# usamec/GAML

Hardware: NVIDIA B200
Metric: alignments_scored_per_s (higher is better)
Workload: dtype f64

## Files before the change

### gaml_b200/csrc/engine.cu

```cuda
#include <cuda_runtime.h>
#include <dlfcn.h>

#include <algorithm>
#include <atomic>
#include <climits>
#include <limits>
#include <cmath>
#include <cstdio>
#include <chrono>
#include <cstring>
#include <memory>
#include <memory_resource>
#include <string>
#include <unordered_map>
#include <unordered_set>
#include <vector>

#include "../../include/gaml_b200.h"
#include "kernels.h"
#include "walk_set.h"

namespace gaml {
namespace {

// ... 950 lines not shown
        CU(rs.d_pairs.reserve((size_t)rs.n_local * 16, 0, false, ctx->stream));
        uint32_t* bad = static_cast<uint32_t*>(ctx->d_csr_temp.p);
        CU(cudaMemsetAsync(bad, 0, 4, ctx->stream));
        launch_pack_pairs(rs.mate[0].first.p, rs.mate[1].first.p, rs.n_local, rs.d_partner12.as<int32_t>(), rs.d_pairs.p, bad, ctx->stream);
        launches++;
        pack_bad = 1;
        CU(cudaMemcpyAsync(&pack_bad, bad, 4, cudaMemcpyDeviceToHost, ctx->stream));
      }
      CU(cudaStreamSynchronize(ctx->stream));
      if (rs.cfg.kind == GAML_KIND_PAIRED && rs.n_mates == 2 && rs.n_local > 0) rs.pairs_ok = pack_bad == 0;
      rs.fast_ok = false;
      if (rs.pairs_ok && rs.comb_ok && rs.lens_uniform && rs.tq_shift > 0) {
        CU(rs.d_fast.reserve((size_t)rs.n_local * 16, 0, false, ctx->stream));
        CU(rs.d_xlist.reserve((size_t)rs.n_local * 4, 0, false, ctx->stream));
        uint32_t* flags = rs.mate[0].cursor.as<uint32_t>();
        CU(build_fast_pairs(rs.d_pairs.p, rs.n_local, rs.tq_shift, rs.ins_n, rs.uniform_ll, rs.d_fast.p, flags, rs.d_xlist.as<uint32_t>(),
                            ctx->d_csr_temp.p, ctx->d_csr_temp.cap, ctx->stream, &launches));
        uint32_t n_cross = 0;
        CU(cudaMemcpyAsync(&n_cross, flags + rs.n_local, 4, cudaMemcpyDeviceToHost, ctx->stream));
        CU(cudaStreamSynchronize(ctx->stream));
        rs.n_cross = (int)n_cross;
        rs.fast_ok = true;
      }
      rs.t2pack_ok = false;
      if (rs.pairs_ok && rs.class_begin[3] > 0) {
        const size_t n0 = (size_t)(rs.class_begin[1] - rs.class_begin[0]), n1 = (size_t)(rs.class_begin[2] - rs.class_begin[1]),
                     n2 = (size_t)(rs.class_begin[3] - rs.class_begin[2]);
        rs.t2base[0] = 0;
        rs.t2base[1] = (uint32_t)(2 * n0);
        rs.t2base[2] = (uint32_t)(2 * n0 + 2 * n1);
        CU(rs.d_t2pack.reserve((2 * n0 + 2 * n1 + 3 * n2) * 16, 0, false, ctx->stream));
        uint32_t* bad = static_cast<uint32_t*>(ctx->d_csr_temp.p);
        CU(cudaMemsetAsync(bad, 0, 4, ctx->stream));
        launch_pack_tier2(rs.d_cdesc.p, rs.mate[0].crows.p, rs.mate[1].crows.p, rs.class_begin, rs.cbase, rs.t2base, rs.d_t2pack.p,
                          bad, ctx->stream);
        launches++;
        uint32_t t2_bad = 1;
        CU(cudaMemcpyAsync(&t2_bad, bad, 4, cudaMemcpyDeviceToHost, ctx->stream));
        CU(cudaStreamSynchronize(ctx->stream));
        rs.t2pack_ok = t2_bad == 0;
      }
      ctx->stats.kernel_launches += launches;
      rs.complex_dirty = false;
      rs.base_built = false;
      if (rs.cfg.kind == GAML_KIND_PAIRED && rs.n_mates == 2 && rs.n_local > 0 && rs.pairs_ok) {
        DevBuf counts;
        CU(counts.reserve((size_t)rs.n_local * 2, 0, false, ctx->stream));
        for (int m = 0; m < 2; m++) {
          MateStore& st = rs.mate[m];
          launch_extract_counts(st.first.p, st.rowptr.as<uint32_t>(), rs.n_local, counts.as<uint16_t>(), ctx->stream);
          st.h_count.resize((size_t)rs.n_local);
          CU(cudaMemcpyAsync(st.h_count.data(), counts.p, (size_t)rs.n_local * 2, cudaMemcpyDeviceToHost, ctx->stream));
          CU(cudaStreamSynchronize(ctx->stream));
          ctx->stats.kernel_launches++;
        }
        CU(rs.d_dirty.reserve((size_t)rs.n_local * 4, 0, false, ctx->stream));
        CU(cudaMemsetAsync(rs.d_dirty.p, 0, (size_t)rs.n_local * 4, ctx->stream));
        rs.h_dirty.assign((size_t)rs.n_local, 0);
        rs.n_appx = 0;
        rs.base_built = true;
      }
    }
    if (pass == 1 || !rs.fast_ok || rs.perm_valid || !ctx->permute_reads) break;
    {
      const int n = rs.n_local;
      DevBuf keys, ids, inv, temp, nf;
      CU(keys.reserve((size_t)n * 2 * 8, 0, false, ctx->stream));
      CU(ids.reserve((size_t)n * 2 * 4, 0, false, ctx->stream));
// ... 2793 lines not shown
```

### gaml_b200/csrc/kernels.cu

```cuda
#include <cub/device/device_radix_sort.cuh>
#include <cub/device/device_scan.cuh>

#include <chrono>
#include <cstdio>
#include <cstdlib>
#include <cstring>
#include <type_traits>
#include <utility>

#include "kernels.h"

namespace gaml {

namespace {

constexpr int kCapLong = 8;
constexpr int kBlock = 256;
constexpr int kOvfBlock = 128;

__device__ __forceinline__ int4 ldg4(const void* p) { return __ldg(reinterpret_cast<const int4*>(p)); }
__device__ __forceinline__ uint4 ldg_stream(const uint4* p) {
  uint4 v;
  asm volatile("ld.global.nc.L1::no_allocate.v4.u32 {%0,%1,%2,%3}, [%4];" : "=r"(v.x), "=r"(v.y), "=r"(v.z), "=r"(v.w) : "l"(p));
  return v;
}
__device__ __forceinline__ void ldg256(const uint4* p, uint4& a, uint4& b) {
  asm volatile("ld.global.nc.v8.u32 {%0,%1,%2,%3,%4,%5,%6,%7}, [%8];"
               : "=r"(a.x), "=r"(a.y), "=r"(a.z), "=r"(a.w), "=r"(b.x), "=r"(b.y), "=r"(b.z), "=r"(b.w) : "l"(p));
}
constexpr int kPackKeyBits = 22;
constexpr uint32_t kPackKeyMask = (1u << kPackKeyBits) - 1u;
constexpr uint32_t kPackEdMask = 0x7fu;

__device__ __forceinline__ int wrap_add(int a, int b) { return (int)((unsigned)a + (unsigned)b); }

__device__ __forceinline__ void pdl_release() { asm volatile("griddepcontrol.launch_dependents;"); }
__device__ __forceinline__ void pdl_wait() { asm volatile("griddepcontrol.wait;" ::: "memory"); }
enum { kTlApply = 0, kTlTier1, kTlTier2, kTlOverflow, kTlDelta, kTlTotal, kTlKernels };
__device__ __forceinline__ unsigned long long global_ns() {
  unsigned long long t;
  asm volatile("mov.u64 %0, %%globaltimer;" : "=l"(t));
  return t;
}
__device__ __forceinline__ void tl_begin(unsigned long long* tl, int k) {
  if (tl && threadIdx.x == 0) atomicMax(tl + 2 * k, ~global_ns());
}
__device__ __forceinline__ void tl_end(unsigned long long* tl, int k) {
  if (tl && threadIdx.x == 0) atomicMax(tl + 2 * k + 1, global_ns());
}
__device__ __forceinline__ void prefetch_l2(const void* p) { asm volatile("prefetch.global.L2 [%0];" ::"l"(p)); }

constexpr double kFixScale = 1099511627776.0;
constexpr double kFixLimit = 4194304.0;

struct Acc {
  unsigned long long lo;
  long long hi;
  unsigned neginf, bad;
};
__device__ __forceinline__ Acc acc_zero() { return Acc{0ull, 0ll, 0u, 0u}; }
__device__ __forceinline__ void acc_add_q(Acc& a, long long q) {
// ... 654 lines not shown
  const RowShort* rows1 = static_cast<const RowShort*>(P.m[0].crows);
  const RowShort* rows2 = static_cast<const RowShort*>(P.m[1].crows);
  const int n_tiles = (P.n_main + kBlock - 1) / kBlock;
  int tile = blockIdx.x, buf = 0;
  for (; tile < n_tiles; __syncthreads(), tile = s_tile[buf], buf ^= 1) {
    if (threadIdx.x == 0) s_tile[buf] = (int)gridDim.x + (int)atomicAdd(P.tile_counter + 2, 1u);
    const int k = tile * kBlock + (int)threadIdx.x;
    if (k >= P.n_main) continue;
    int cls = 0;
#pragma unroll
    for (int c = 1; c < 5; c++) cls += (k >= P.class_begin[c]) ? 1 : 0;
    const uint32_t j = (uint32_t)(k - P.class_begin[cls]);
    const int4 dsc = ldg4(static_cast<const int4*>(P.cdesc) + k);
    const int r = dsc.x;
    const uint32_t ll = (uint32_t)dsc.y;
    double acc;
    int st;
    switch (cls) {
      case 0: st = tier2_read<1, 2>(P, rows1, rows2, P.cbase[0][0] + j, P.cbase[1][0] + 2 * j, ll, acc); break;
      case 1: st = tier2_read<2, 1>(P, rows1, rows2, P.cbase[0][1] + 2 * j, P.cbase[1][1] + j, ll, acc); break;
      case 2: st = tier2_read<2, 2>(P, rows1, rows2, P.cbase[0][2] + 2 * j, P.cbase[1][2] + 2 * j, ll, acc); break;
      default: st = 1; acc = 0.0; break;
    }
    if (P.dirty && __ldg(P.dirty + r)) continue;
    if (st > 0) {
      P.values[r] = acc;
      acc_read(P, sum, floored, acc, (ll & 0xffff) + (ll >> 16));
    } else if (st < 0) {
      push_overflow(P, r);
    }
  }
}

struct Rec8 { uint32_t w; int pos; };
__device__ __forceinline__ Rec8 rec8(uint32_t a, uint32_t b) { return Rec8{a, (int)b}; }

template <int N1, int N2>
__device__ __forceinline__ int tier2_packed_read(const ScoreParams& P, const int4* __restrict__ sa1, const int4* __restrict__ sa2,
                                                 const Rec8 (&x)[2], const Rec8 (&y)[2], uint32_t ll, double& acc, long long& qv) {
  const int l1 = ll & 0xffff, l2 = ll >> 16;
  int4 ox[2], oy[2];
#pragma unroll
  for (int i = 0; i < 2; i++) {
    ox[i] = __ldg(sa1 + (x[i < N1 ? i : 0].w & kPackKeyMask));
    oy[i] = __ldg(sa2 + (y[i < N2 ? i : 0].w & kPackKeyMask));
  }
  int ex[2], ey[2];
#pragma unroll
  for (int i = 0; i < 2; i++) {
    ex[i] = (int)((x[i < N1 ? i : 0].w >> kPackKeyBits) & kPackEdMask);
    ey[i] = (int)((y[i < N2 ? i : 0].w >> kPackKeyBits) & kPackEdMask);
  }
  const TermEntry* __restrict__ tq = P.tq ? static_cast<const TermEntry*>(P.tq) + 1 : nullptr;
  double px[2], py[2];
  if (!tq) {
#pragma unroll
    for (int i = 0; i < 2; i++) {
      px[i] = __dmul_rn(__ldg(P.m[0].pow_mismatch + ex[i]), __ldg(P.m[0].pow_match + (l1 - ex[i])));
      py[i] = __dmul_rn(__ldg(P.m[1].pow_mismatch + ey[i]), __ldg(P.m[1].pow_match + (l2 - ey[i])));
    }
  }
  bool lx[2], ly[2], multi = false;
  int wx[2], wy[2], qx[2], qy[2], orx[2], ory[2];
#pragma unroll
  for (int i = 0; i < 2; i++) {
    const uint32_t fx = (uint32_t)ox[i].x, fy = (uint32_t)oy[i].x;
    const bool hx = i < N1, hy = i < N2;
    const bool vx = hx && (fx & 0x7fffffffu) == P.epoch, vy = hy && (fy & 0x7fffffffu) == P.epoch;
    multi |= (vx && (fx >> 31)) || (vy && (fy >> 31));
    wx[i] = ox[i].y; wy[i] = oy[i].y;
    qx[i] = wrap_add(x[hx ? i : 0].pos, ox[i].z); qy[i] = wrap_add(y[hy ? i : 0].pos, oy[i].z);
    lx[i] = vx && qx[i] >= ox[i].w;
    ly[i] = vy && qy[i] >= oy[i].w;
    orx[i] = (int)((x[hx ? i : 0].w >> 29) & 1u); ory[i] = (int)((y[hy ? i : 0].w >> 29) & 1u);
  }
  bool order = false;
  if (N1 > 1) {
    const bool dup = lx[0] && lx[1] && wx[0] == wx[1] && qx[0] == qx[1];
    const bool same = ((x[0].w ^ x[1].w) >> kPackKeyBits) == 0u;
    order |= dup && !same;
    lx[1] = lx[1] && !dup;
  }
  if (N2 > 1) {
    const bool dup = ly[0] && ly[1] && wy[0] == wy[1] && qy[0] == qy[1];
    const bool same = ((y[0].w ^ y[1].w) >> kPackKeyBits) == 0u;
    order |= dup && !same;
    ly[1] = ly[1] && !dup;
  }
  bool ok[2][2];
  int dist[2][2];
  int nt = 0, nok = 0;
#pragma unroll
  for (int i = 0; i < N1; i++) {
#pragma unroll
    for (int j = 0; j < N2; j++) {
      const bool fwd = qx[i] < qy[j];
      const int d = fwd ? qy[j] - qx[i] + l2 : qx[i] - qy[j] + l1;
      const bool term = lx[i] && ly[j] && wx[i] == wy[j] && orx[i] != ory[j] && orx[i] == (fwd ? 0 : 1);
      nt += term ? 1 : 0;
      ok[i][j] = term && (unsigned)d < (unsigned)P.ins_n;
      nok += ok[i][j] ? 1 : 0;
      dist[i][j] = ok[i][j] ? d : 0;
    }
  }
  double t[2][2];
  long long tqv[2][2];
  if (tq) {
    const int lim = 1 << P.tq_shift;
    bool untab = false;
    TermEntry e[2][2];
#pragma unroll
    for (int i = 0; i < N1; i++) {
#pragma unroll
      for (int j = 0; j < N2; j++) {
        const bool fit = ex[i] < lim && ey[j] < lim;
        untab |= ok[i][j] && !fit;
        const size_t idx = fit ? (size_t)((ex[i] << P.tq_shift) | ey[j]) * (size_t)P.ins_n + (size_t)dist[i][j] : 0;
        const int4 w = __ldg(reinterpret_cast<const int4*>(tq + idx));
        e[i][j].t = __hiloint2double(w.y, w.x);
        e[i][j].q = (long long)(((unsigned long long)(uint32_t)w.w << 32) | (uint32_t)w.z);
      }
    }
#pragma unroll
    for (int i = 0; i < N1; i++) {
#pragma unroll
      for (int j = 0; j < N2; j++) { t[i][j] = e[i][j].t; tqv[i][j] = e[i][j].q; }
    }
    if (untab) {
#pragma unroll
      for (int i = 0; i < N1; i++) {
#pragma unroll
        for (int j = 0; j < N2; j++) {
          if (ok[i][j] && !(ex[i] < lim && ey[j] < lim)) {
            t[i][j] = __dmul_rn(__dmul_rn(__ldg(P.uni_prob[0] + ex[i]), __ldg(P.uni_prob[1] + ey[j])), __ldg(P.ins_tab + dist[i][j]));
            tqv[i][j] = kTermOdd;
          }
        }
      }
    }
  } else {
#pragma unroll
    for (int i = 0; i < N1; i++) {
#pragma unroll
      for (int j = 0; j < N2; j++) {
        t[i][j] = __dmul_rn(__dmul_rn(px[i], py[j]), __ldg(P.ins_tab + dist[i][j]));
        tqv[i][j] = kTermOdd;
      }
    }
  }
  acc = 0.0;
  qv = kTermOdd;
#pragma unroll
  for (int i = 0; i < N1; i++) {
#pragma unroll
    for (int j = 0; j < N2; j++) {
      acc = __dadd_rn(acc, ok[i][j] ? t[i][j] : 0.0);
      if (ok[i][j] && nok == 1) qv = tqv[i][j];
    }
  }
  return multi ? 0 : ((order || nt > 2) ? -1 : 1);
}

__device__ __forceinline__ void acc_term_known(Acc& a, unsigned& floored, const double2* log_tab, double p, long long qv,
                                               double pstar, long long qthr) {
  if (p < pstar) {
    floored++;
    acc_add_q(a, qthr);
  } else if (qv != kTermOdd) {
    acc_add_q(a, qv);
  } else {
    const double lg = table_log(log_tab, p);
    if (fabs(lg) < kFixLimit) acc_add_q(a, __double2ll_rn(lg * kFixScale));
    else acc_count_odd(a, lg);
  }
}

__device__ __forceinline__ void tier2_packed_tiles(const ScoreParams& P, int* s_tile, Acc& sum, unsigned& floored) {
  const int4* sa1 = reinterpret_cast<const int4*>(P.m[0].slots_a);
  const int4* sa2 = reinterpret_cast<const int4*>(P.m[1].slots_a);
  const double2* log_tab = static_cast<const double2*>(P.log_tab);
  const uint4* __restrict__ pk = static_cast<const uint4*>(P.t2pack);
  const int n_tiles = (P.n_main + kBlock - 1) / kBlock;
  int tile = blockIdx.x, buf = 0;
  for (; tile < n_tiles; __syncthreads(), tile = s_tile[buf], buf ^= 1) {
    if (threadIdx.x == 0) s_tile[buf] = (int)gridDim.x + (int)atomicAdd(P.tile_counter + 2, 1u);
    const int k = tile * kBlock + (int)threadIdx.x;
    if (k >= P.n_main) continue;
    int cls = 0;
#pragma unroll
    for (int c = 1; c < 5; c++) cls += (k >= P.class_begin[c]) ? 1 : 0;
    const uint32_t j = (uint32_t)(k - P.class_begin[cls]);
    int r, st;
    uint32_t ll;
    double acc = 0.0;
    long long qv = kTermOdd;
    if (cls < 3) {
      const uint32_t n_c = (uint32_t)(P.class_begin[cls + 1] - P.class_begin[cls]);
      const uint4* base = pk + P.t2base[cls];
      const uint4 u0 = ldg_stream(base + j), u1 = ldg_stream(base + n_c + j);
      r = (int)u0.x;
      ll = u0.y;
      if (cls == 0) {
        const Rec8 x[2] = {rec8(u0.z, u0.w), rec8(u0.z, u0.w)}, y[2] = {rec8(u1.x, u1.y), rec8(u1.z, u1.w)};
        st = tier2_packed_read<1, 2>(P, sa1, sa2, x, y, ll, acc, qv);
      } else if (cls == 1) {
        const Rec8 x[2] = {rec8(u1.x, u1.y), rec8(u1.z, u1.w)}, y[2] = {rec8(u0.z, u0.w), rec8(u0.z, u0.w)};
        st = tier2_packed_read<2, 1>(P, sa1, sa2, x, y, ll, acc, qv);
      } else {
        const uint4 u2 = ldg_stream(base + 2 * n_c + j);
        const Rec8 x[2] = {rec8(u1.x, u1.y), rec8(u1.z, u1.w)}, y[2] = {rec8(u2.x, u2.y), rec8(u2.z, u2.w)};
        st = tier2_packed_read<2, 2>(P, sa1, sa2, x, y, ll, acc, qv);
      }
    } else {
      const int4 dsc = ldg4(static_cast<const int4*>(P.cdesc) + k);
      r = dsc.x;
      ll = (uint32_t)dsc.y;
      st = 1;
    }
    if (P.dirty && __ldg(P.dirty + r)) continue;
    if (st > 0) {
      P.values[r] = acc;
      double pstar;
      long long qthr;
      term_consts(P, (ll & 0xffff) + (ll >> 16), pstar, qthr);
      acc_term_known(sum, floored, log_tab, acc, qv, pstar, qthr);
    } else if (st < 0) {
      push_overflow(P, r);
    }
  }
}

struct TwoLive { Placed1 p0, p1; int n; bool multi, order; };
__device__ __forceinline__ void two_live_scan(const ScoreParams& P, int m, const RowShort* __restrict__ rows, uint32_t b,
                                              uint32_t n, TwoLive& t) {
  t.n = 0;
  t.multi = t.order = false;
  t.p0 = t.p1 = Placed1{false, false, 0, 0, 0};
  for (uint32_t i = 0; i < n; i += 2) {
    const int4 r0 = ldg4(rows + b + i), r1 = i + 1 < n ? ldg4(rows + b + i + 1) : r0;
    Placed1 q[2] = {place_row(P, m, r0), place_row(P, m, r1)};
    if (i + 1 >= n) q[1].live = q[1].multi = false;
#pragma unroll
    for (int j = 0; j < 2; j++) {
      if (!q[j].live) continue;
      t.multi |= q[j].multi;
      if (t.n > 0 && t.p0.walk == q[j].walk && t.p0.pos == q[j].pos) {
        if (t.p0.edor != q[j].edor) t.order = true;
      } else if (t.n > 1 && t.p1.walk == q[j].walk && t.p1.pos == q[j].pos) {
        if (t.p1.edor != q[j].edor) t.order = true;
      } else if (t.n == 0) {
        t.p0 = q[j];
        t.n = 1;
      } else if (t.n == 1) {
        t.p1 = q[j];
        t.n = 2;
      } else {
        t.order = true;
      }
    }
  }
}
// ... 398 lines not shown
      __syncthreads();
#pragma unroll
      for (int j = 0; j < kR; j++) u_cur[j] = u_nxt[j];
      tile = next;
      next = s_tile[buf];
      buf ^= 1;
    }
  } else {
    while (tile < n_tiles) {
      if (threadIdx.x == 0) s_tile[buf] = 2 * (int)gridDim.x + (int)atomicAdd(P.tile_counter, 1u);
      prefetch_tile(next);
      tier1_body<kCov, kPacked, false, kR>(P, src1, src2, lane, sa1, sa2, log_tab, tile * kTile + wib * (32 * kR), n, sum, floored);
      __syncthreads();
      tile = next;
      next = s_tile[buf];
      buf ^= 1;
    }
  }
  if (kPhase != 1 && kTab && P.n_cross > 0) {
    const uint4* __restrict__ pairs = static_cast<const uint4*>(P.pairs);
    constexpr int kXR = 2, kXTile = kXR * kBlock;
    const int x_tiles = (P.n_cross + kXTile - 1) / kXTile;
    __syncthreads();
    int xt = blockIdx.x, xbuf = 0;
    for (; xt < x_tiles; __syncthreads(), xt = s_tile[xbuf], xbuf ^= 1) {
      if (threadIdx.x == 0) s_tile[xbuf] = (int)gridDim.x + (int)atomicAdd(P.tile_counter + 3, 1u);
      tier1_body<false, true, kTab, kXR>(P, pairs, src2, lane, sa1, sa2, log_tab, xt * kXTile + wib * (32 * kXR), P.n_cross, sum, floored, P.xlist);
    }
  }
  if (kPhase != 2) tl_end(P.timeline, kTlTier1);
  if (kPhase != 1 && P.n_main > 0) {
    __syncthreads();
    if (kPhase == 0) tl_begin(P.timeline, kTlTier2);
    if (!kCov && P.t2pack) tier2_packed_tiles(P, s_tile, sum, floored);
    else tier2_tiles(P, s_tile, sum, floored);
  }
  if (kPhase != 1) tl_end(P.timeline, kTlTier2);
  if (!P.chain_first) pdl_wait();
  block_accumulate(sum, floored, P.accum);
  if (P.finish_here) finish_set_if_complete(P);
}


__device__ __forceinline__ bool paired_read_any(const ScoreParams& P, int r, uint32_t ll, double& acc) {
  if (paired_read_ordered(P, r, acc)) return true;
  const int n1 = gather_short(P.m[0], P.epoch, r, nullptr), n2 = gather_short(P.m[1], P.epoch, r, nullptr);
  const unsigned long long base = atomicAdd(P.scratch_cursor, (unsigned long long)(n1 + n2));
  if (base + n1 + n2 > P.scratch_cap) {
    atomicOr(P.error_flag, 2u);
    return false;
  }
  Plc* a = P.scratch + base;
  Plc* b = a + n1;
  gather_short(P.m[0], P.epoch, r, a);
  gather_short(P.m[1], P.epoch, r, b);
  acc = apply_pairs(P, a, n1, b, n2, ll & 0xffff, ll >> 16, acc, P.n_erased);
  return true;
}

__global__ void __launch_bounds__(kOvfBlock) paired_multi_kernel(const ScoreParams P) {
  tl_begin(P.timeline, kTlDelta);
  if (P.chain_first) pdl_wait();
  pdl_release();
  Acc sum = acc_zero();
  unsigned floored = 0;
  const uint32_t total = P.n_mtouch > 0 ? __ldg(P.mtouch_prefix + P.n_mtouch) : 0u;
  for (uint32_t q = blockIdx.x * blockDim.x + threadIdx.x; q < total; q += gridDim.x * blockDim.x) {
// ... 1416 lines not shown
  batch_finalize_kernel<<<(B.n_cand + 127) / 128, 128, 0, st>>>(B, out, error_flag, (long long)P.n_reads);
  if (timing) {
    cudaEventRecord(ev[4], st);
    cudaEventSynchronize(ev[4]);
    float t[4];
    for (int i = 0; i < 4; i++) cudaEventElapsedTime(&t[i], ev[i], ev[i + 1]);
    fprintf(stderr, "[gaml_b200 batch] n_len %d: base %.3f ms, prefix %.3f ms, touch %.3f ms (%u records), finalize %.3f ms\n", B.n_len, t[0], t[1],
            t[2], n_touch_records, t[3]);
    for (auto& e : ev) cudaEventDestroy(e);
  }
}
int batch_hist_bins(int n_len) { return ((n_len + kBatchMaxLen - 1) / kBatchMaxLen) * (kBatchMaxLen + 1); }
int batch_launches(int n_len, bool touch) { return 2 * ((n_len + kBatchMaxLen - 1) / kBatchMaxLen) + (touch ? 1 : 0) + 1; }

__global__ void build_term_table_kernel(const double* p1, const double* p2, const double* ins, int ins_n, int shift, const double2* log_tab,
                                        TermEntry* out) {
  const size_t total = ((size_t)1 << (2 * shift)) * (size_t)ins_n;
  for (size_t i = blockIdx.x * (size_t)blockDim.x + threadIdx.x; i < total; i += (size_t)gridDim.x * blockDim.x) {
    const int d = (int)(i % (size_t)ins_n);
    const int ee = (int)(i / (size_t)ins_n);
    const int e1 = ee >> shift, e2 = ee & ((1 << shift) - 1);
    const double t = __dmul_rn(__dmul_rn(p1[e1], p2[e2]), ins[d]);
    out[i + 1] = TermEntry{t, fix_log(log_tab, t)};
    if (i == 0) out[0] = TermEntry{0.0, kTermOdd};
  }
}
void launch_build_term_table(const double* p1, const double* p2, const double* ins, int ins_n, int shift, const void* log_tab, void* out,
                             int sm_count, cudaStream_t st) {
  const size_t total = ((size_t)1 << (2 * shift)) * (size_t)ins_n;
  build_term_table_kernel<<<grid_for(total, 256, sm_count, 8), 256, 0, st>>>(p1, p2, ins, ins_n, shift, static_cast<const double2*>(log_tab),
                                                                           static_cast<TermEntry*>(out));
}

__global__ void pack_fast_kernel(const uint4* pairs, int n, int shift, int ins_n, uint32_t uniform_ll, uint4* out, uint32_t* flags) {
  const int r = blockIdx.x * blockDim.x + threadIdx.x;
  if (r > n) return;
  if (r == n) { flags[r] = 0u; return; }
  const uint4 pr = pairs[r];
  const uint32_t key1 = pr.x & kPackKeyMask;
  const int e1 = (int)((pr.x >> kPackKeyBits) & kPackEdMask), e2 = (int)((pr.y >> kPackKeyBits) & kPackEdMask);
  const int xo = (int)((pr.x >> 29) & 1u), yo = (int)((pr.y >> 29) & 1u);
  const bool none = ((pr.x >> 30) & 1u) != 0u || ((pr.y >> 30) & 1u) != 0u;
  const bool tier2 = (pr.x >> 31) != 0u, same = (pr.y >> 31) != 0u;
  const int pos1 = (int)pr.z, pos2 = (int)pr.w;
  const int l1 = (int)(uniform_ll & 0xffff), l2 = (int)(uniform_ll >> 16);
  const bool fit = e1 < (1 << shift) && e2 < (1 << shift);
  uint4 v = make_uint4(0u, 0u, 0u, 0u);
  uint32_t cross = 0u;
  uint32_t tix = 0u;
  if (!none && same && fit) {
    const bool fwd = pos1 < pos2;
    const int d = fwd ? pos2 - pos1 + l2 : pos1 - pos2 + l1;
    const bool term = xo != yo && xo == (fwd ? 0 : 1) && (unsigned)d < (unsigned)ins_n;
    tix = term ? 1u + (uint32_t)((e1 << shift) | e2) * (uint32_t)ins_n + (uint32_t)d : 0u;
  }
  if (tier2) {
    v.x = 0x80000000u | key1;
    v.w = tix;
  } else if (none) {
    v.x = 0x40000000u;
  } else if (!same || !fit) {
    v.x = 0x80000000u | key1;
    cross = 1u;
  } else {
    v.x = key1;
    v.y = (uint32_t)pos1;
    v.z = (uint32_t)pos2;
    v.w = tix;
  }
  out[r] = v;
  flags[r] = cross;
}
__global__ void perm_keys_kernel(const uint4* fast, int n, unsigned long long* keys, uint32_t* ids) {
  const int r = blockIdx.x * blockDim.x + threadIdx.x;
  if (r >= n) return;
  const uint4 f = fast[r];
  const bool elsewhere = (f.x >> 31) != 0u, noterm = ((f.x >> 30) & 1u) != 0u;
  unsigned long long k;
  if (elsewhere) k = (1ull << 63) | ((unsigned long long)(f.x & 0x3fffffffu) << 32) | (unsigned long long)f.w;
  else if (noterm) k = (0x3fffffffull << 32) | (unsigned long long)(uint32_t)r;
  else k = ((unsigned long long)(f.x & 0x3fffffffu) << 32) | (unsigned long long)f.w;
  keys[r] = k;
  ids[r] = (uint32_t)r;
}
__global__ void perm_finish_kernel(const unsigned long long* sorted_keys, const uint32_t* sorted_ids, int n, uint32_t* inv, uint32_t* n_fast) {
  const int i = blockIdx.x * blockDim.x + threadIdx.x;
  if (i >= n) return;
  inv[sorted_ids[i]] = (uint32_t)i;
// ... 34 lines not shown
}
cudaError_t build_fast_pairs(const void* pairs, int n, int shift, int ins_n, uint32_t uniform_ll, void* fast, uint32_t* flags, uint32_t* list,
                             void* temp, size_t temp_bytes, cudaStream_t st, int* launches) {
  pack_fast_kernel<<<(n + 1 + 255) / 256, 256, 0, st>>>(static_cast<const uint4*>(pairs), n, shift, ins_n, uniform_ll, static_cast<uint4*>(fast), flags);
  size_t need = 0;
  cub::DeviceScan::ExclusiveSum(nullptr, need, flags, flags, n + 1, st);
  if (need > temp_bytes) return cudaErrorMemoryAllocation;
  cudaError_t err = cub::DeviceScan::ExclusiveSum(temp, need, flags, flags, n + 1, st);
  if (err != cudaSuccess) return err;
  scatter_flagged_kernel<<<(n + 255) / 256, 256, 0, st>>>(flags, n, list);
  (*launches) += 3;
  return cudaGetLastError();
}

__global__ void pack_pairs_kernel(const int4* first1, const int4* first2, int n, const int32_t* partner12, uint4* out, uint32_t* bad) {
  const int r = blockIdx.x * blockDim.x + threadIdx.x;
  if (r >= n) return;
  const int4 a = ldg4(first1 + r), b = ldg4(first2 + r);
  const bool none1 = a.x < 0, none2 = b.x < 0;
  const uint32_t k1 = none1 ? 0u : (uint32_t)a.x, k2 = none2 ? 0u : (uint32_t)b.x;
  const uint32_t ed1 = (uint32_t)a.z & 0xffffu, ed2 = (uint32_t)b.z & 0xffffu;
  if (k1 > kPackKeyMask || k2 > kPackKeyMask || ed1 > kPackEdMask || ed2 > kPackEdMask) *bad = 1u;
  const uint32_t tier2 = ((((uint32_t)a.z | (uint32_t)b.z) >> 17) & 0x1fffu) != 0u ? 1u : 0u;
  uint4 v;
  v.x = (k1 & kPackKeyMask) | ((ed1 & kPackEdMask) << kPackKeyBits) | ((((uint32_t)a.z >> 30) & 1u) << 29) | ((none1 ? 1u : 0u) << 30) | (tier2 << 31);
  const uint32_t same = (partner12 && !none1 && !none2 && partner12[k1] == (int32_t)k2) ? 1u : 0u;
  v.y = (k2 & kPackKeyMask) | ((ed2 & kPackEdMask) << kPackKeyBits) | ((((uint32_t)b.z >> 30) & 1u) << 29) | ((none2 ? 1u : 0u) << 30) | (same << 31);
  v.z = (uint32_t)a.y;
  v.w = (uint32_t)b.y;
  out[r] = v;
}
__global__ void pack_tier2_kernel(const int4* cdesc, const RowShort* rows1, const RowShort* rows2, int n_entries, int b1, int b2,
                                  uint32_t cb1_0, uint32_t cb1_1, uint32_t cb1_2, uint32_t cb2_0, uint32_t cb2_1, uint32_t cb2_2,
                                  uint32_t tb0, uint32_t tb1, uint32_t tb2, uint4* out, uint32_t* bad) {
  const int k = blockIdx.x * blockDim.x + threadIdx.x;
  if (k >= n_entries) return;
  const int cls = (k >= b1 ? 1 : 0) + (k >= b2 ? 1 : 0);
  const int cb = cls == 0 ? 0 : (cls == 1 ? b1 : b2);
  const uint32_t n_c = (uint32_t)((cls == 0 ? b1 : (cls == 1 ? b2 : n_entries)) - cb);
  const uint32_t j = (uint32_t)(k - cb);
  const int n1 = cls == 0 ? 1 : 2, n2 = cls == 1 ? 1 : 2;
  const uint32_t r1 = (cls == 0 ? cb1_0 : (cls == 1 ? cb1_1 : cb1_2)) + (uint32_t)n1 * j;
  const uint32_t r2 = (cls == 0 ? cb2_0 : (cls == 1 ? cb2_1 : cb2_2)) + (uint32_t)n2 * j;
  const uint32_t tb = cls == 0 ? tb0 : (cls == 1 ? tb1 : tb2);
  bool unfit = false;
  auto pack = [&](const RowShort& rw, uint32_t& a, uint32_t& b) {
    const uint32_t ed = (uint32_t)rw.edor & 0xffffu;
    if (rw.key < 0 || (uint32_t)rw.key > kPackKeyMask || ed > kPackEdMask) unfit = true;
    a = ((uint32_t)rw.key & kPackKeyMask) | ((ed & kPackEdMask) << kPackKeyBits) | ((((uint32_t)rw.edor >> 30) & 1u) << 29);
    b = (uint32_t)rw.pos;
  };
  const int4 dsc = cdesc[k];
  uint4 u0, u1, u2;
  u0.x = (uint32_t)dsc.x; u0.y = (uint32_t)dsc.y; u0.z = u0.w = 0u;
  const RowShort x0 = rows1[r1], x1 = rows1[r1 + (n1 > 1 ? 1 : 0)], y0 = rows2[r2], y1 = rows2[r2 + (n2 > 1 ? 1 : 0)];
  if (cls == 0) {
    pack(x0, u0.z, u0.w); pack(y0, u1.x, u1.y); pack(y1, u1.z, u1.w);
  } else if (cls == 1) {
    pack(y0, u0.z, u0.w); pack(x0, u1.x, u1.y); pack(x1, u1.z, u1.w);
  } else {
    pack(x0, u1.x, u1.y); pack(x1, u1.z, u1.w); pack(y0, u2.x, u2.y); pack(y1, u2.z, u2.w);
    out[tb + 2 * n_c + j] = u2;
  }
  out[tb + j] = u0;
  out[tb + n_c + j] = u1;
  if (unfit) *bad = 1u;
}
void launch_pack_tier2(const void* cdesc, const void* rows1, const void* rows2, const int32_t* class_begin, const uint32_t cbase[2][5],
                       const uint32_t tbase[3], void* out, uint32_t* bad, cudaStream_t st) {
  const int n = class_begin[3];
  if (n > 0)
    pack_tier2_kernel<<<(n + 255) / 256, 256, 0, st>>>(static_cast<const int4*>(cdesc), static_cast<const RowShort*>(rows1),
                                                       static_cast<const RowShort*>(rows2), n, class_begin[1], class_begin[2],
                                                       cbase[0][0], cbase[0][1], cbase[0][2], cbase[1][0], cbase[1][1], cbase[1][2],
                                                       tbase[0], tbase[1], tbase[2], static_cast<uint4*>(out), bad);
}

void launch_pack_pairs(const void* first1, const void* first2, int n, const int32_t* partner12, void* out, uint32_t* bad, cudaStream_t st) {
  if (n > 0)
    pack_pairs_kernel<<<(n + 255) / 256, 256, 0, st>>>(static_cast<const int4*>(first1), static_cast<const int4*>(first2), n,
                                                       partner12, static_cast<uint4*>(out), bad);
}

void launch_cdesc_fill(const uint32_t* list, int n_complex, const uint32_t* lens, const uint32_t* cptr1, const uint32_t* cptr2,
                       void* desc, cudaStream_t st) {
  if (n_complex > 0)
    cdesc_fill_kernel<<<(n_complex + 255) / 256, 256, 0, st>>>(list, n_complex, lens, cptr1, cptr2, static_cast<int4*>(desc));
}

size_t coverage_sort_temp_bytes(unsigned n) {
  size_t need = 0;
  cub::DeviceRadixSort::SortKeys(nullptr, need, (const unsigned long long*)nullptr, (unsigned long long*)nullptr, (int)n);
  return need;
}

cudaError_t launch_coverage(const unsigned long long* keys_in, unsigned long long* keys_sorted, unsigned n, void* temp,
                            size_t temp_bytes, const int* cs_begin, const int* cs, double step, double min_from_start, int* bad,
                            int sm_count, cudaStream_t st) {
  size_t need = temp_bytes;
  cudaError_t err = cub::DeviceRadixSort::SortKeys(temp, need, keys_in, keys_sorted, (int)n, 0, 64, st);
  if (err != cudaSuccess) return err;
  coverage_sweep_kernel<<<grid_for(n, 256, sm_count, 8), 256, 0, st>>>(keys_sorted, n, cs_begin, cs, step, min_from_start, bad);
  return cudaGetLastError();
}

void launch_pacbio_alnprob(const AlnProbParams& A, int sm_count, cudaStream_t st) {
  const int grid = grid_for((size_t)A.n, 128, sm_count, 8);
  pacbio_alnprob_kernel<<<grid, 128, 0, st>>>(A);
// ... 59 lines not shown
```

### gaml_b200/csrc/kernels.h

```cpp
#pragma once
#include <cuda_runtime.h>

#include "device_types.h"

namespace gaml {

struct PendingLaunch {
  const void* func = nullptr;
  unsigned grid = 1, block = 1;
  bool pdl = false;
  int n_args = 0;
  void* arg_ptrs[16];
  alignas(16) unsigned char arg_buf[1536];
};
struct LaunchList {
  PendingLaunch item[16];
  int n = 0;
};
void set_launch_recorder(LaunchList* list);
cudaError_t issue_launch(const PendingLaunch& pl, cudaStream_t st);

enum { kGridPairedFull = 0, kGridPairedComplex, kGridPairedTotal, kGridSingleFull, kGridSingleComplex, kGridPacbioFull };
int score_grid(int which, int n_items, int sm_count);
int overflow_grid(int sm_count);

constexpr int kInlineStores = 8;
struct StoreTables {
  SlotA* a[kInlineStores];
  SlotB* b[kInlineStores];
  SlotA* cb[kInlineStores];
  const int32_t* cm[kInlineStores];
};
void launch_apply_slots(const SlotUpdate* upd, int n, const SlotUpdate* patch, int n_patch, const int32_t* skip, int n_skip,
                        SlotA* const* tab_a, SlotB* const* tab_b, SlotA* const* comb_base,
                        const int32_t* const* comb_map, const StoreTables* inline_tabs, uint32_t epoch, unsigned long long* flags,
                        int n_flag_words, unsigned long long* timeline, cudaStream_t st);
constexpr int kTimelineWords = 12;
int launch_paired_full(const ScoreParams& P, int grid, int cgrid, uint32_t n_multi_items, int ovf_grid, int sm_count,
                       cudaStream_t st, bool chained, bool profile, cudaEvent_t e0, cudaEvent_t e1,
                       bool tail);
void launch_paired_tail(const ScoreParams& P, int ovf_grid, cudaStream_t st);
void launch_paired_delta(const ScoreParams& P, uint32_t n_touch_records, int grid_total, int ovf_grid, int sm_count, cudaStream_t st,
                         bool chained, bool profile, cudaEvent_t e0, cudaEvent_t e1);
void launch_single_full(const ScoreParams& P, int grid, int cgrid, int ovf_grid, cudaStream_t st, bool chained, bool profile,
                        cudaEvent_t e0, cudaEvent_t e1);
void launch_pacbio_full(const ScoreParams& P, int grid, int ovf_grid, cudaStream_t st, bool chained, bool profile, cudaEvent_t e0,
                        cudaEvent_t e1);

cudaError_t build_csr(const void* arena, size_t n_records, int n_reads, bool is_long, uint32_t* rowptr, uint32_t* cursor,
                      void* rows, void* first, void* temp, size_t temp_bytes, int sm_count, cudaStream_t st, int* launches);
cudaError_t build_complex_list(const void* first1, const void* first2, int n_reads, uint32_t* flags, uint32_t* list,
                               void* temp, size_t temp_bytes, cudaStream_t st, int* launches, uint32_t* n_complex_out,
                               int32_t* class_begin);
void launch_pack_tier2(const void* cdesc, const void* rows1, const void* rows2, const int32_t* class_begin, const uint32_t cbase[2][5],
                       const uint32_t tbase[3], void* out, uint32_t* bad, cudaStream_t st);
void launch_pack_pairs(const void* first1, const void* first2, int n, const int32_t* partner12, void* out, uint32_t* bad, cudaStream_t st);
void launch_cdesc_fill(const uint32_t* list, int n_complex, const uint32_t* lens, const uint32_t* cptr1, const uint32_t* cptr2,
                       void* desc, cudaStream_t st);
cudaError_t compact_offsets(const uint32_t* list, int n_complex, const uint32_t* rowptr, uint32_t* cptr, const uint32_t* lens,
                            uint32_t* clens, void* temp, size_t temp_bytes, cudaStream_t st, int* launches);
cudaError_t compact_copy(const uint32_t* list, int n_complex, const uint32_t* rowptr, const uint32_t* cptr, const void* rows,
                         void* crows, cudaStream_t st, int* launches);
void launch_batch(const ScoreParams& P, const BatchParams& B, uint32_t n_touch_records, double* out, const uint32_t* error_flag,
                  int sm_count, cudaStream_t st);
int batch_hist_bins(int n_len);
int batch_launches(int n_len, bool touch);
void launch_build_term_table(const double* p1, const double* p2, const double* ins, int ins_n, int shift, const void* log_tab, void* out,
                             int sm_count, cudaStream_t st);
cudaError_t build_fast_pairs(const void* pairs, int n, int shift, int ins_n, uint32_t uniform_ll, void* fast, uint32_t* flags, uint32_t* list,
                             void* temp, size_t temp_bytes, cudaStream_t st, int* launches);
struct AppendGroupHost { uint32_t read, new_begin, n_new, dst; };
struct AppendMate {
  const void* arena_src; void* arena_dst; uint32_t n_rec;
  const void* groups; int n_groups; const void* new_rows; void* rows; void* first;
};
struct AppendJob {
  AppendMate m[2];
  uint32_t* dirty; void* pairs; void* fast;
  const uint32_t* appx_src; uint32_t* appx_dst; int n_appx_new;
  const int2* p12_patch; int n_p12; int32_t* p12;
  const int2* p21_patch; int n_p21; int32_t* p21;
};
void launch_append_apply(const AppendJob& J, cudaStream_t st);
void launch_extract_counts(const void* first, const uint32_t* rowptr, int n, uint16_t* out, cudaStream_t st);
size_t perm_temp_bytes(int n);
cudaError_t build_read_permutation(const void* fast, int n, unsigned long long* keys, uint32_t* ids, uint32_t* inv, uint32_t* n_fast,
                                   void* temp, size_t temp_bytes, cudaStream_t st, int* launches);
void launch_remap_arena(void* arena, size_t n_records, const uint32_t* inv, int sm_count, cudaStream_t st);
// ... 16 lines not shown
```

Before: 143.3 billion.

## Precompute static partner-pair term index into tier-2 packed entries

At pack time, the tier-2 packing kernel finds the alignment pair whose keys are statically partnered and stores a flag, combination index, term bit and term-table index in the entry word that used to hold the lengths. At scoring time with the term table enabled, that pair's slot data comes from a combined 32-byte record and its term entry from the precomputed index, so the per-pair orientation and distance checks and the dependent table lookup are skipped. The scoring loop is also split into separate load and entry helpers and specialised on whether the table is used. This adds pack-time work and more branching, and relies on the uniform read-length assumption staying valid.

New measurement: 132.1 billion, median of 6. -7.8%, worse.

```diff
diff --git a/gaml_b200/csrc/engine.cu b/gaml_b200/csrc/engine.cu
--- a/gaml_b200/csrc/engine.cu
+++ b/gaml_b200/csrc/engine.cu
@@ -1006,8 +1006,9 @@
         CU(rs.d_t2pack.reserve((2 * n0 + 2 * n1 + 3 * n2) * 16, 0, false, ctx->stream));
         uint32_t* bad = static_cast<uint32_t*>(ctx->d_csr_temp.p);
         CU(cudaMemsetAsync(bad, 0, 4, ctx->stream));
-        launch_pack_tier2(rs.d_cdesc.p, rs.mate[0].crows.p, rs.mate[1].crows.p, rs.class_begin, rs.cbase, rs.t2base, rs.d_t2pack.p,
-                          bad, ctx->stream);
+        launch_pack_tier2(rs.d_cdesc.p, rs.mate[0].crows.p, rs.mate[1].crows.p, rs.class_begin, rs.cbase, rs.t2base,
+                          rs.d_partner12.as<int32_t>(), rs.fast_ok ? rs.tq_shift : 0, rs.ins_n, rs.uniform_ll, rs.d_t2pack.p, bad,
+                          ctx->stream);
         launches++;
         uint32_t t2_bad = 1;
         CU(cudaMemcpyAsync(&t2_bad, bad, 4, cudaMemcpyDeviceToHost, ctx->stream));
diff --git a/gaml_b200/csrc/kernels.cu b/gaml_b200/csrc/kernels.cu
--- a/gaml_b200/csrc/kernels.cu
+++ b/gaml_b200/csrc/kernels.cu
@@ -27,6 +27,11 @@
 __device__ __forceinline__ void ldg256(const uint4* p, uint4& a, uint4& b) {
   asm volatile("ld.global.nc.v8.u32 {%0,%1,%2,%3,%4,%5,%6,%7}, [%8];"
                : "=r"(a.x), "=r"(a.y), "=r"(a.z), "=r"(a.w), "=r"(b.x), "=r"(b.y), "=r"(b.z), "=r"(b.w) : "l"(p));
+}
+__device__ __forceinline__ int4 ldg_nc(const int4* p) {
+  int4 v;
+  asm volatile("ld.global.nc.v4.s32 {%0,%1,%2,%3}, [%4];" : "=r"(v.x), "=r"(v.y), "=r"(v.z), "=r"(v.w) : "l"(p));
+  return v;
 }
 constexpr int kPackKeyBits = 22;
 constexpr uint32_t kPackKeyMask = (1u << kPackKeyBits) - 1u;
@@ -747,18 +752,42 @@
   }
 }
 
+constexpr uint32_t kT2TixMask = (1u << 21) - 1u;
+constexpr int kT2CombShift = 21;
+constexpr uint32_t kT2Static = 1u << 23;
+constexpr uint32_t kT2Term = 1u << 24;
 struct Rec8 { uint32_t w; int pos; };
 __device__ __forceinline__ Rec8 rec8(uint32_t a, uint32_t b) { return Rec8{a, (int)b}; }
 
-template <int N1, int N2>
-__device__ __forceinline__ int tier2_packed_read(const ScoreParams& P, const int4* __restrict__ sa1, const int4* __restrict__ sa2,
-                                                 const Rec8 (&x)[2], const Rec8 (&y)[2], uint32_t ll, double& acc, long long& qv) {
+template <bool kTab, int N1, int N2>
+__device__ __forceinline__ int tier2_packed_read(const ScoreParams& P, const Rec8 (&x)[2], const Rec8 (&y)[2], uint32_t sw, uint32_t ll,
+                                                 double& acc, long long& qv) {
+  const int4* __restrict__ sa1 = reinterpret_cast<const int4*>(P.m[0].slots_a);
+  const int4* __restrict__ sa2 = reinterpret_cast<const int4*>(P.m[1].slots_a);
+  const int4* __restrict__ tq = static_cast<const int4*>(P.tq);
   const int l1 = ll & 0xffff, l2 = ll >> 16;
+  const bool hs = kTab && (sw & kT2Static) != 0u;
+  const int si = (int)((sw >> (kT2CombShift + 1)) & 1u), sj = (int)((sw >> kT2CombShift) & 1u);
+  int4 cx = make_int4(0, 0, 0, 0), cy = cx, ts = cx, gx[2] = {cx, cx}, gy[2] = {cx, cx};
+  if (kTab) {
+    ts = ldg_nc(tq + (sw & kT2TixMask));
+    if (hs) {
+      uint4 a, b;
+      ldg256(static_cast<const uint4*>(P.comb) + 4 * ((si ? x[1].w : x[0].w) & kPackKeyMask), a, b);
+      cx = make_int4((int)a.x, (int)a.y, (int)a.z, (int)a.w);
+      cy = make_int4((int)b.x, (int)b.y, (int)b.z, (int)b.w);
+    }
+  }
+#pragma unroll
+  for (int i = 0; i < 2; i++) {
+    if (i < N1 && !(hs && si == i)) gx[i] = ldg_nc(sa1 + (x[i].w & kPackKeyMask));
+    if (i < N2 && !(hs && sj == i)) gy[i] = ldg_nc(sa2 + (y[i].w & kPackKeyMask));
+  }
   int4 ox[2], oy[2];
 #pragma unroll
   for (int i = 0; i < 2; i++) {
-    ox[i] = __ldg(sa1 + (x[i < N1 ? i : 0].w & kPackKeyMask));
-    oy[i] = __ldg(sa2 + (y[i < N2 ? i : 0].w & kPackKeyMask));
+    ox[i] = i < N1 ? (hs && si == i ? cx : gx[i]) : gx[0];
+    oy[i] = i < N2 ? (hs && sj == i ? cy : gy[i]) : gy[0];
   }
   int ex[2], ey[2];
 #pragma unroll
@@ -766,9 +795,8 @@
     ex[i] = (int)((x[i < N1 ? i : 0].w >> kPackKeyBits) & kPackEdMask);
     ey[i] = (int)((y[i < N2 ? i : 0].w >> kPackKeyBits) & kPackEdMask);
   }
-  const TermEntry* __restrict__ tq = P.tq ? static_cast<const TermEntry*>(P.tq) + 1 : nullptr;
   double px[2], py[2];
-  if (!tq) {
+  if (!kTab) {
 #pragma unroll
     for (int i = 0; i < 2; i++) {
       px[i] = __dmul_rn(__ldg(P.m[0].pow_mismatch + ex[i]), __ldg(P.m[0].pow_match + (l1 - ex[i])));
@@ -809,44 +837,44 @@
   for (int i = 0; i < N1; i++) {
 #pragma unroll
     for (int j = 0; j < N2; j++) {
+      const bool stc = hs && si == i && sj == j;
       const bool fwd = qx[i] < qy[j];
       const int d = fwd ? qy[j] - qx[i] + l2 : qx[i] - qy[j] + l1;
-      const bool term = lx[i] && ly[j] && wx[i] == wy[j] && orx[i] != ory[j] && orx[i] == (fwd ? 0 : 1);
+      const bool filt = stc ? (sw & kT2Term) != 0u : orx[i] != ory[j] && orx[i] == (fwd ? 0 : 1);
+      const bool term = lx[i] && ly[j] && wx[i] == wy[j] && filt;
       nt += term ? 1 : 0;
-      ok[i][j] = term && (unsigned)d < (unsigned)P.ins_n;
+      ok[i][j] = term && (stc ? (sw & kT2TixMask) != 0u : (unsigned)d < (unsigned)P.ins_n);
       nok += ok[i][j] ? 1 : 0;
       dist[i][j] = ok[i][j] ? d : 0;
     }
   }
   double t[2][2];
   long long tqv[2][2];
-  if (tq) {
+  if (kTab) {
     const int lim = 1 << P.tq_shift;
     bool untab = false;
-    TermEntry e[2][2];
 #pragma unroll
     for (int i = 0; i < N1; i++) {
 #pragma unroll
       for (int j = 0; j < N2; j++) {
+        const bool stc = hs && si == i && sj == j;
         const bool fit = ex[i] < lim && ey[j] < lim;
-        untab |= ok[i][j] && !fit;
-        const size_t idx = fit ? (size_t)((ex[i] << P.tq_shift) | ey[j]) * (size_t)P.ins_n + (size_t)dist[i][j] : 0;
-        const int4 w = __ldg(reinterpret_cast<const int4*>(tq + idx));
-        e[i][j].t = __hiloint2double(w.y, w.x);
-        e[i][j].q = (long long)(((unsigned long long)(uint32_t)w.w << 32) | (uint32_t)w.z);
+        untab |= ok[i][j] && !stc && !fit;
+        int4 w = ts;
+        if (!stc) {
+          w = make_int4(0, 0, 0, 0);
+          if (ok[i][j] && fit) w = __ldg(tq + 1 + (size_t)((ex[i] << P.tq_shift) | ey[j]) * (size_t)P.ins_n + (size_t)dist[i][j]);
+        }
+        t[i][j] = __hiloint2double(w.y, w.x);
+        tqv[i][j] = (long long)(((unsigned long long)(uint32_t)w.w << 32) | (uint32_t)w.z);
       }
     }
-#pragma unroll
-    for (int i = 0; i < N1; i++) {
-#pragma unroll
-      for (int j = 0; j < N2; j++) { t[i][j] = e[i][j].t; tqv[i][j] = e[i][j].q; }
-    }
     if (untab) {
 #pragma unroll
       for (int i = 0; i < N1; i++) {
 #pragma unroll
         for (int j = 0; j < N2; j++) {
-          if (ok[i][j] && !(ex[i] < lim && ey[j] < lim)) {
+          if (ok[i][j] && !(hs && si == i && sj == j) && !(ex[i] < lim && ey[j] < lim)) {
             t[i][j] = __dmul_rn(__dmul_rn(__ldg(P.uni_prob[0] + ex[i]), __ldg(P.uni_prob[1] + ey[j])), __ldg(P.ins_tab + dist[i][j]));
             tqv[i][j] = kTermOdd;
           }
@@ -890,58 +918,72 @@
   }
 }
 
+__device__ __forceinline__ int tier2_class(const ScoreParams& P, int k) {
+  int cls = 0;
+#pragma unroll
+  for (int c = 1; c < 5; c++) cls += (k >= P.class_begin[c]) ? 1 : 0;
+  return cls;
+}
+__device__ __forceinline__ void tier2_load(const ScoreParams& P, int k, uint4 (&u)[2]) {
+  k = min(k, P.n_main - 1);
+  const int cls = tier2_class(P, k);
+  const uint32_t j = (uint32_t)(k - P.class_begin[cls]);
+  if (cls < 3) {
+    const uint32_t n_c = (uint32_t)(P.class_begin[cls + 1] - P.class_begin[cls]);
+    const uint4* base = static_cast<const uint4*>(P.t2pack) + P.t2base[cls];
+    u[0] = ldg_stream(base + j);
+    u[1] = ldg_stream(base + n_c + j);
+  } else {
+    u[0] = ldg_stream(static_cast<const uint4*>(P.cdesc) + k);
+    u[1] = u[0];
+  }
+}
+template <bool kTab>
+__device__ __forceinline__ void tier2_entry(const ScoreParams& P, const uint4 (&u)[2], int k, Acc& sum, unsigned& floored,
+                                            const double2* log_tab) {
+  if (k >= P.n_main) return;
+  const int cls = tier2_class(P, k);
+  const int r = (int)u[0].x;
+  const uint32_t ll = kTab ? P.uniform_ll : u[0].y;
+  const bool dirty = P.dirty && __ldg(P.dirty + r);
+  double acc = 0.0;
+  long long qv = kTermOdd;
+  int st = 1;
+  if (cls == 0) {
+    const Rec8 x[2] = {rec8(u[0].z, u[0].w), rec8(u[0].z, u[0].w)}, y[2] = {rec8(u[1].x, u[1].y), rec8(u[1].z, u[1].w)};
+    st = tier2_packed_read<kTab, 1, 2>(P, x, y, u[0].y, ll, acc, qv);
+  } else if (cls == 1) {
+    const Rec8 x[2] = {rec8(u[1].x, u[1].y), rec8(u[1].z, u[1].w)}, y[2] = {rec8(u[0].z, u[0].w), rec8(u[0].z, u[0].w)};
+    st = tier2_packed_read<kTab, 2, 1>(P, x, y, u[0].y, ll, acc, qv);
+  } else if (cls == 2) {
+    const uint32_t n_c = (uint32_t)(P.class_begin[3] - P.class_begin[2]);
+    const uint4 u2 = ldg_stream(static_cast<const uint4*>(P.t2pack) + P.t2base[2] + 2 * n_c + (uint32_t)(k - P.class_begin[2]));
+    const Rec8 x[2] = {rec8(u[1].x, u[1].y), rec8(u[1].z, u[1].w)}, y[2] = {rec8(u2.x, u2.y), rec8(u2.z, u2.w)};
+    st = tier2_packed_read<kTab, 2, 2>(P, x, y, u[0].y, ll, acc, qv);
+  }
+  if (dirty) return;
+  if (st > 0) {
+    P.values[r] = acc;
+    double pstar = P.uni_pstar;
+    long long qthr = P.uni_qthr;
+    if (!kTab) term_consts(P, (ll & 0xffff) + (ll >> 16), pstar, qthr);
+    acc_term_known(sum, floored, log_tab, acc, qv, pstar, qthr);
+  } else if (st < 0) {
+    push_overflow(P, r);
+  }
+}
+
+template <bool kTab>
 __device__ __forceinline__ void tier2_packed_tiles(const ScoreParams& P, int* s_tile, Acc& sum, unsigned& floored) {
-  const int4* sa1 = reinterpret_cast<const int4*>(P.m[0].slots_a);
-  const int4* sa2 = reinterpret_cast<const int4*>(P.m[1].slots_a);
   const double2* log_tab = static_cast<const double2*>(P.log_tab);
-  const uint4* __restrict__ pk = static_cast<const uint4*>(P.t2pack);
   const int n_tiles = (P.n_main + kBlock - 1) / kBlock;
   int tile = blockIdx.x, buf = 0;
   for (; tile < n_tiles; __syncthreads(), tile = s_tile[buf], buf ^= 1) {
     if (threadIdx.x == 0) s_tile[buf] = (int)gridDim.x + (int)atomicAdd(P.tile_counter + 2, 1u);
     const int k = tile * kBlock + (int)threadIdx.x;
-    if (k >= P.n_main) continue;
-    int cls = 0;
-#pragma unroll
-    for (int c = 1; c < 5; c++) cls += (k >= P.class_begin[c]) ? 1 : 0;
-    const uint32_t j = (uint32_t)(k - P.class_begin[cls]);
-    int r, st;
-    uint32_t ll;
-    double acc = 0.0;
-    long long qv = kTermOdd;
-    if (cls < 3) {
-      const uint32_t n_c = (uint32_t)(P.class_begin[cls + 1] - P.class_begin[cls]);
-      const uint4* base = pk + P.t2base[cls];
-      const uint4 u0 = ldg_stream(base + j), u1 = ldg_stream(base + n_c + j);
-      r = (int)u0.x;
-      ll = u0.y;
-      if (cls == 0) {
-        const Rec8 x[2] = {rec8(u0.z, u0.w), rec8(u0.z, u0.w)}, y[2] = {rec8(u1.x, u1.y), rec8(u1.z, u1.w)};
-        st = tier2_packed_read<1, 2>(P, sa1, sa2, x, y, ll, acc, qv);
-      } else if (cls == 1) {
-        const Rec8 x[2] = {rec8(u1.x, u1.y), rec8(u1.z, u1.w)}, y[2] = {rec8(u0.z, u0.w), rec8(u0.z, u0.w)};
-        st = tier2_packed_read<2, 1>(P, sa1, sa2, x, y, ll, acc, qv);
-      } else {
-        const uint4 u2 = ldg_stream(base + 2 * n_c + j);
-        const Rec8 x[2] = {rec8(u1.x, u1.y), rec8(u1.z, u1.w)}, y[2] = {rec8(u2.x, u2.y), rec8(u2.z, u2.w)};
-        st = tier2_packed_read<2, 2>(P, sa1, sa2, x, y, ll, acc, qv);
-      }
-    } else {
-      const int4 dsc = ldg4(static_cast<const int4*>(P.cdesc) + k);
-      r = dsc.x;
-      ll = (uint32_t)dsc.y;
-      st = 1;
-    }
-    if (P.dirty && __ldg(P.dirty + r)) continue;
-    if (st > 0) {
-      P.values[r] = acc;
-      double pstar;
-      long long qthr;
-      term_consts(P, (ll & 0xffff) + (ll >> 16), pstar, qthr);
-      acc_term_known(sum, floored, log_tab, acc, qv, pstar, qthr);
-    } else if (st < 0) {
-      push_overflow(P, r);
-    }
+    uint4 u[2];
+    tier2_load(P, k, u);
+    tier2_entry<kTab>(P, u, k, sum, floored, log_tab);
   }
 }
 
@@ -1406,7 +1448,7 @@
   if (kPhase != 1 && P.n_main > 0) {
     __syncthreads();
     if (kPhase == 0) tl_begin(P.timeline, kTlTier2);
-    if (!kCov && P.t2pack) tier2_packed_tiles(P, s_tile, sum, floored);
+    if (!kCov && P.t2pack) tier2_packed_tiles<kTab>(P, s_tile, sum, floored);
     else tier2_tiles(P, s_tile, sum, floored);
   }
   if (kPhase != 1) tl_end(P.timeline, kTlTier2);
@@ -2889,6 +2931,17 @@
                                                                            static_cast<TermEntry*>(out));
 }
 
+struct StaticTerm { bool term; uint32_t tix; };
+__device__ __forceinline__ StaticTerm static_term(int pos1, int e1, int o1, int pos2, int e2, int o2, uint32_t uniform_ll, int shift,
+                                                  int ins_n) {
+  const int l1 = (int)(uniform_ll & 0xffff), l2 = (int)(uniform_ll >> 16);
+  const bool fwd = pos1 < pos2;
+  const int d = fwd ? pos2 - pos1 + l2 : pos1 - pos2 + l1;
+  const bool term = o1 != o2 && o1 == (fwd ? 0 : 1);
+  const uint32_t tix = term && (unsigned)d < (unsigned)ins_n ? 1u + (uint32_t)((e1 << shift) | e2) * (uint32_t)ins_n + (uint32_t)d : 0u;
+  return StaticTerm{term, tix};
+}
+
 __global__ void pack_fast_kernel(const uint4* pairs, int n, int shift, int ins_n, uint32_t uniform_ll, uint4* out, uint32_t* flags) {
   const int r = blockIdx.x * blockDim.x + threadIdx.x;
   if (r > n) return;
@@ -2900,17 +2953,11 @@
   const bool none = ((pr.x >> 30) & 1u) != 0u || ((pr.y >> 30) & 1u) != 0u;
   const bool tier2 = (pr.x >> 31) != 0u, same = (pr.y >> 31) != 0u;
   const int pos1 = (int)pr.z, pos2 = (int)pr.w;
-  const int l1 = (int)(uniform_ll & 0xffff), l2 = (int)(uniform_ll >> 16);
   const bool fit = e1 < (1 << shift) && e2 < (1 << shift);
   uint4 v = make_uint4(0u, 0u, 0u, 0u);
   uint32_t cross = 0u;
   uint32_t tix = 0u;
-  if (!none && same && fit) {
-    const bool fwd = pos1 < pos2;
-    const int d = fwd ? pos2 - pos1 + l2 : pos1 - pos2 + l1;
-    const bool term = xo != yo && xo == (fwd ? 0 : 1) && (unsigned)d < (unsigned)ins_n;
-    tix = term ? 1u + (uint32_t)((e1 << shift) | e2) * (uint32_t)ins_n + (uint32_t)d : 0u;
-  }
+  if (!none && same && fit) tix = static_term(pos1, e1, xo, pos2, e2, yo, uniform_ll, shift, ins_n).tix;
   if (tier2) {
     v.x = 0x80000000u | key1;
     v.w = tix;
@@ -3011,7 +3058,8 @@
 }
 __global__ void pack_tier2_kernel(const int4* cdesc, const RowShort* rows1, const RowShort* rows2, int n_entries, int b1, int b2,
                                   uint32_t cb1_0, uint32_t cb1_1, uint32_t cb1_2, uint32_t cb2_0, uint32_t cb2_1, uint32_t cb2_2,
-                                  uint32_t tb0, uint32_t tb1, uint32_t tb2, uint4* out, uint32_t* bad) {
+                                  uint32_t tb0, uint32_t tb1, uint32_t tb2, const int32_t* partner12, int shift, int ins_n,
+                                  uint32_t uniform_ll, uint4* out, uint32_t* bad) {
   const int k = blockIdx.x * blockDim.x + threadIdx.x;
   if (k >= n_entries) return;
   const int cls = (k >= b1 ? 1 : 0) + (k >= b2 ? 1 : 0);
@@ -3033,6 +3081,21 @@
   uint4 u0, u1, u2;
   u0.x = (uint32_t)dsc.x; u0.y = (uint32_t)dsc.y; u0.z = u0.w = 0u;
   const RowShort x0 = rows1[r1], x1 = rows1[r1 + (n1 > 1 ? 1 : 0)], y0 = rows2[r2], y1 = rows2[r2 + (n2 > 1 ? 1 : 0)];
+  if (shift > 0) {
+    uint32_t sw = 0u;
+    auto try_static = [&](const RowShort& a, const RowShort& b, uint32_t c) {
+      if (sw != 0u || a.key < 0 || b.key < 0 || partner12[a.key] != b.key) return;
+      const int e1 = a.edor & 0xffff, e2 = b.edor & 0xffff;
+      if (e1 >= (1 << shift) || e2 >= (1 << shift)) return;
+      const StaticTerm s = static_term(a.pos, e1, (a.edor >> 30) & 1, b.pos, e2, (b.edor >> 30) & 1, uniform_ll, shift, ins_n);
+      sw = kT2Static | (c << kT2CombShift) | (s.term ? kT2Term : 0u) | s.tix;
+    };
+    try_static(x0, y0, 0u);
+    if (n2 > 1) try_static(x0, y1, 1u);
+    if (n1 > 1) try_static(x1, y0, 2u);
+    if (n1 > 1 && n2 > 1) try_static(x1, y1, 3u);
+    u0.y = sw;
+  }
   if (cls == 0) {
     pack(x0, u0.z, u0.w); pack(y0, u1.x, u1.y); pack(y1, u1.z, u1.w);
   } else if (cls == 1) {
@@ -3046,13 +3109,15 @@
   if (unfit) *bad = 1u;
 }
 void launch_pack_tier2(const void* cdesc, const void* rows1, const void* rows2, const int32_t* class_begin, const uint32_t cbase[2][5],
-                       const uint32_t tbase[3], void* out, uint32_t* bad, cudaStream_t st) {
+                       const uint32_t tbase[3], const int32_t* partner12, int shift, int ins_n, uint32_t uniform_ll, void* out,
+                       uint32_t* bad, cudaStream_t st) {
   const int n = class_begin[3];
   if (n > 0)
     pack_tier2_kernel<<<(n + 255) / 256, 256, 0, st>>>(static_cast<const int4*>(cdesc), static_cast<const RowShort*>(rows1),
                                                        static_cast<const RowShort*>(rows2), n, class_begin[1], class_begin[2],
                                                        cbase[0][0], cbase[0][1], cbase[0][2], cbase[1][0], cbase[1][1], cbase[1][2],
-                                                       tbase[0], tbase[1], tbase[2], static_cast<uint4*>(out), bad);
+                                                       tbase[0], tbase[1], tbase[2], partner12, shift, ins_n, uniform_ll,
+                                                       static_cast<uint4*>(out), bad);
 }
 
 void launch_pack_pairs(const void* first1, const void* first2, int n, const int32_t* partner12, void* out, uint32_t* bad, cudaStream_t st) {
diff --git a/gaml_b200/csrc/kernels.h b/gaml_b200/csrc/kernels.h
--- a/gaml_b200/csrc/kernels.h
+++ b/gaml_b200/csrc/kernels.h
@@ -53,7 +53,8 @@
                                void* temp, size_t temp_bytes, cudaStream_t st, int* launches, uint32_t* n_complex_out,
                                int32_t* class_begin);
 void launch_pack_tier2(const void* cdesc, const void* rows1, const void* rows2, const int32_t* class_begin, const uint32_t cbase[2][5],
-                       const uint32_t tbase[3], void* out, uint32_t* bad, cudaStream_t st);
+                       const uint32_t tbase[3], const int32_t* partner12, int shift, int ins_n, uint32_t uniform_ll, void* out,
+                       uint32_t* bad, cudaStream_t st);
 void launch_pack_pairs(const void* first1, const void* first2, int n, const int32_t* partner12, void* out, uint32_t* bad, cudaStream_t st);
 void launch_cdesc_fill(const uint32_t* list, int n_complex, const uint32_t* lens, const uint32_t* cptr1, const uint32_t* cptr2,
                        void* desc, cudaStream_t st);
```
